# EricssonResearch/Robust-Tracking-MPC-over-Lossy-Networks

Measured on AMD Instinct MI355X. Metric: QP solves/sec (= MPC steps/sec) at batch, higher is better.
Workload: dtype f64

## Files before the change

### robust-tracking-mpc-over-lossy-networks_amd/csrc/tmpc_kernels.hip

```cpp
#ifdef TMPC_HOST_SIM
#include "hip_sim.hpp"
#else
#include <hip/hip_runtime.h>
#endif

#include <algorithm>
#include <cmath>
#include <cstdint>
#include <string>
#include <type_traits>
#include <utility>

#include "tmpc_device.hpp"
#include "tmpc_launch.hpp"
#include "tmpc_wave.hpp"
#include "tmpc_mc_step.hpp"

namespace tmpc {

namespace {

using wv::WAVE;
using wv::fast_rcp;
using wv::readlane_d;
// ... 212 lines not shown
        int ks = 0;
        for (; ks + 1 < nks; ks += 2) {
            fetch(D1, t1, g1);
            multiply(std::integral_constant<int, 0>{}, D0, t0, g0);
            fetch(D0, t0, g0);
            multiply(std::integral_constant<int, NACC - 1>{}, D1, t1, g1);
        }
        if (ks < nks) multiply(std::integral_constant<int, 0>{}, D0, t0, g0);
    }
    static_assert(WaveLds<SH>::RED >= 2 * (SH::NDP + 4), "look-ahead of the MFMA pass stays inside the transposition tile");
    double *mtk = mt + kq * SH::LDM + c;
#pragma unroll
    for (int I = 0; I < NB; ++I)
#pragma unroll
        for (int J = 0; J <= I; ++J)
#pragma unroll
            for (int reg = 0; reg < 4; ++reg) {
                const int row = 16 * I + kq + 4 * reg, col = 16 * J + c;
                double v = acc[0][I * (I + 1) / 2 + J][reg];
                if constexpr (NACC == 2) v += acc[1][I * (I + 1) / 2 + J][reg];
                if (row < NV && col < NV) {
                    mtk[(16 * I + 4 * reg) * SH::LDM + 16 * J] = v;
                    if (I != J) mt[col * SH::LDM + row] = v;
                }
                if (I == IT && row == NV && col < NV) gdr[col] = v;
            }
    wave_lds_fence();
}

template <class SH>
__device__ __forceinline__ void sweep_a_factored(const double *Hct, const double (&s)[SH::RS], const double (&lam)[SH::RS],
                                                 const double *rpw, double (&rs)[SH::RS], double &gap_l, double &rpn_l, double obj_l,
                                                 double *red, double *csums, int lane) {
    constexpr int KC = SH::KC, KT = SH::KT, NCCP = SH::NCCP;
    double acc[KT + KC + 2];
    static_for<SH::FC>([&](auto kc_) {
        constexpr int kc = decltype(kc_)::value;
        const int r = lane + kc * WAVE;
        double hc[KC];
#pragma unroll
        for (int a = 0; a < KC; ++a) hc[a] = Hct[a * NCCP + r];
        double D = 0.0, t = 0.0;
#pragma unroll
        for (int sd = 0; sd < SH::csides(kc); ++sd) {
            constexpr int base = SH::cbase(kc);
            const int i = base + sd;
            const double rsi = fast_rcp(s[i]);
            rs[i] = rsi;
            const double d = lam[i] * rsi;
            const double rpi = rpw[i * WAVE + lane];
            gap_l = fma(s[i], lam[i], gap_l);
            rpn_l = vmax_abs(rpn_l, rpi);
            D += d;
            t = sd ? fma(-d, rpi, t) : fma(d, rpi, t);
        }
#pragma unroll
        for (int a = 0; a < KC; ++a) {
            const double dg = D * hc[a];
#pragma unroll
            for (int b2 = a; b2 < KC; ++b2) acc[col_off<KC>(a) + b2 - a] = kc == 0 ? dg * hc[b2] : fma(dg, hc[b2], acc[col_off<KC>(a) + b2 - a]);
            acc[KT + a] = kc == 0 ? hc[a] * t : fma(hc[a], t, acc[KT + a]);
        }
    });
    acc[KT + KC] = gap_l;
    acc[KT + KC + 1] = obj_l;
    wave_sums_to_lds<SH, KT + KC + 2>(acc, red, csums, lane);
}

struct McNone {};
struct McStepArg {
    const McFused *rec;
    int t;
    uint8_t *gamma_out;
};
template <int FUSED> using McArg = std::conditional_t<FUSED == 1, const McFused *, std::conditional_t<FUSED == 2, McStepArg, McNone>>;
#if defined(TMPC_HOST_SIM)
typedef const McFused *McRecord;
__device__ __forceinline__ McRecord mc_record(const McFused *p) { return p; }
#else
typedef const __attribute__((address_space(4))) McFused *McRecord;
__device__ __forceinline__ McRecord mc_record(const McFused *p) {
    unsigned lo = static_cast<unsigned>(reinterpret_cast<uintptr_t>(p)), hi = static_cast<unsigned>(reinterpret_cast<uintptr_t>(p) >> 32);
    asm volatile("" : "+v"(lo), "+v"(hi));
    lo = __builtin_amdgcn_readfirstlane(lo);
    hi = __builtin_amdgcn_readfirstlane(hi);
    return (McRecord)((static_cast<uintptr_t>(hi) << 32) | lo);
}
#endif

template <int NV, int DP, int DS, int KC, int CP, int CS, int WPB, int FUSED>
__device__ __forceinline__ void solve_body(
    const DeviceQP &qp, const int variant_id, const int64_t B,
    const double *__restrict__ x_k, const double *__restrict__ ref, const uint8_t *__restrict__ variant,
    double *__restrict__ u_nom, double *__restrict__ x_nom0, double *__restrict__ xu_ss,
    double *__restrict__ x_nom, int32_t *__restrict__ status, int32_t *__restrict__ iters,
    const int32_t *ws_in, int32_t *ws_out, unsigned long long *__restrict__ next_item,
    const McArg<FUSED> mc) {
    using SH = Shape<NV, DP, DS, KC, CP, CS, tile_rows(NV, WPB)>;
    using WL = WaveLds<SH>;
    constexpr int RS = SH::RS, FD = SH::FD, FC = SH::FC, NDP = SH::NDP, NCCP = SH::NCCP, KT = SH::KT, WCAP = SH::WCAP, LDG = SH::LDG;
#ifdef TMPC_HOST_SIM
    double *smem = sim::lds<double>();
#else
    extern __shared__ __attribute__((aligned(16))) double smem[];
#endif
    double *wbase = smem;
    double *Hct = wbase + WPB * WL::TOTAL;
    double *Psi = Hct + KC * NCCP;
    double *Hs = Psi + KC * NV;
    double *Hinv = Hs + NV * SH::LDH;
    double *Gt = Hinv + NV * SH::LDH;
    const int grows = 4 * qp.nks;

    const int tid = threadIdx.x;
    const int lane_k = tid & (WAVE - 1);
    int lane = lane_k;
    const int wave = __builtin_amdgcn_readfirstlane(tid >> 6);
    const int nx = qp.nx, nu = qp.nu, N = qp.N, nc = qp.nc;

    for (int i = tid; i < (grows + ZERO_ROWS) * LDG; i += blockDim.x) Gt[i] = (i < grows * LDG) ? qp.Gt[i] : 0.0;
    for (int i = tid; i < KC * NCCP; i += blockDim.x) Hct[i] = qp.Hct[i];
    for (int i = tid; i < KC * NV; i += blockDim.x) Psi[i] = qp.Psi[i];
    for (int i = tid; i < NV * NV; i += blockDim.x) { const int r_ = i / NV, c_ = i - r_ * NV; Hs[r_ * SH::LDH + c_] = qp.Hs[i]; Hinv[r_ * SH::LDH + c_] = qp.Hinv[i]; }
    __syncthreads();

    double *red = wbase + wave * WL::TOTAL;
    double *sums = red + WL::BIG;
    double *csums = sums + WL::SUMS;
    double *Pm = csums + WL::CSUMS;
    double *hw = Pm + WL::PMAT;
    double *vec = hw + WL::HROW;
    double *dtw = red;
    double *Mf = red + WL::RED;
    unsigned *park = reinterpret_cast<unsigned *>(red + WL::POL);
    double *qv = vec;
    double *zv = vec + NV;
    double *cgv = vec + 2 * NV;
    double *xin = vec + 3 * NV;
    double *tv = vec + 3 * NV + 32;
    double *uv = vec + 4 * NV + 32;
    double *dzav = vec + 5 * NV + 32;
    double *dzv = vec + 6 * NV + 32;
    double *czv = vec + 7 * NV + 32;
    double *cdzav = czv + 8;
    double *cdzv = czv + 16;

    const int vmask_k = static_cast<int>(qp.vmask[lane]);
    unsigned vmask = static_cast<unsigned>(vmask_k);
    auto valid = [&](int i) { return ((vmask >> i) & 1u) != 0u; };
#define TMPC_REFRESH() do { lane = fresh(lane_k); vmask = static_cast<unsigned>(fresh(vmask_k)); } while (0)

    const int64_t n_waves = static_cast<int64_t>(gridDim.x) * WPB;
    bool first_item = true;
    for (;;) {
        int64_t b;
        if (first_item) {
            b = B < n_waves ? static_cast<int64_t>(wave) * gridDim.x + blockIdx.x : static_cast<int64_t>(blockIdx.x) * WPB + wave;
            first_item = false;
        } else {
            unsigned long long drawn = ~0ull >> 2;
            if (lane_k == 0) {
                const unsigned long long seen = __hip_atomic_load(next_item, __ATOMIC_RELAXED, __HIP_MEMORY_SCOPE_AGENT);
                if (n_waves + static_cast<int64_t>(seen) < B) drawn = atomicAdd(next_item, 1ull);
            }
            b = n_waves + static_cast<int64_t>((static_cast<unsigned long long>(static_cast<unsigned>(__builtin_amdgcn_readfirstlane(static_cast<int>(drawn >> 32)))) << 32) |
                                               static_cast<unsigned>(__builtin_amdgcn_readfirstlane(static_cast<int>(drawn & 0xffffffffull))));
        }
        if (b >= B) break;
        if (variant != nullptr && variant[b] != variant_id) continue;
        if (variant == nullptr && variant_id != 0) continue;

        int n_steps = 1;
        if constexpr (FUSED == 1) n_steps = mc_record(mc)->T;
        for (int t_mc = 0; t_mc < n_steps; ++t_mc) {
        TMPC_REFRESH();
        if constexpr (FUSED != 0) {
            McRecord mr;
            if constexpr (FUSED == 1) mr = mc_record(mc); else mr = mc_record(mc.rec);
            const double *xh = mr->st.x_hat, *rk = mr->st.ref_k;
            if (lane < nx) { xin[lane] = xh[b * nx + lane]; xin[nx + lane] = rk[b * nx + lane]; }
        } else {
            if (lane < nx) { xin[lane] = x_k[b * nx + lane]; xin[nx + lane] = ref[b * nx + lane]; }
        }
        wave_lds_fence();
        int st = TMPC_STATUS_MAX_ITER;
        int it_done = 0;
#ifdef TMPC_ITERS_TOTAL
        int n_reruns = 0, n_rounds = 0, amb_level = 0;
#endif
        const long long t_begin = qp.ticks ? static_cast<long long>(__builtin_amdgcn_s_memrealtime()) : 0;
#ifdef TMPC_STAMPS
        long long tph[16] = {0, 0, 0, 0, 0, 0, 0, 0, 0, 0, 0, 0, 0, 0, 0, 0};
        long long tlast = __builtin_amdgcn_s_memtime();
#endif
        bool infeasible_par = qp.always_infeasible != 0;
        for (int r = lane; r < qp.npar; r += WAVE) {
            double v = qp.gp0[r];
            for (int c = 0; c < nx; ++c) v += qp.Ep[r * nx + c] * xin[c];
            if (v < -1e-9 * (1.0 + fabs(qp.gp0[r]))) infeasible_par = true;
        }
        infeasible_par = __any(infeasible_par);

        if (lane < NV) {
            double v = 0.0;
            if (lane < qp.nv)
                for (int c = 0; c < nx; ++c) v += qp.F1s[lane * nx + c] * xin[c] + qp.F2s[lane * nx + c] * xin[nx + c];
            qv[lane] = v;
        }
        auto compute_h = [&]() {
            TMPC_REFRESH();
            double hv[RS];
            const double *__restrict__ E0 = qp.Esp + lane;
            constexpr size_t PL = static_cast<size_t>(RS) * WAVE;
            for (int c0 = 0; c0 < nx; c0 += 4) {
                double ev[4][RS];
#pragma unroll
                for (int u = 0; u < 4; ++u) {
                    const size_t cu = static_cast<size_t>(c0 + u < nx ? c0 + u : nx - 1);
#pragma unroll
                    for (int i = 0; i < RS; ++i) ev[u][i] = E0[cu * PL + i * WAVE];
                }
                if (c0 == 0) {
#pragma unroll
                    for (int i = 0; i < RS; ++i) hv[i] = qp.g0p[i * WAVE + lane];
                }
#pragma unroll
                for (int u = 0; u < 4; ++u) {
                    const double xc = c0 + u < nx ? xin[c0 + u] : 0.0;
#pragma unroll
                    for (int i = 0; i < RS; ++i) hv[i] = fma(ev[u][i], xc, hv[i]);
                }
            }
            double hmax = 1.0;
#pragma unroll
            for (int i = 0; i < RS; ++i) {
                if (valid(i)) hmax = fmax(hmax, fabs(hv[i]));
                hw[i * WAVE + lane] = hv[i];
            }
            wave_lds_fence();
            return hmax;
        };
        const double hn = wave_max(compute_h());
        double qn = 1.0;
#pragma unroll
        for (int j = 0; j < NV; ++j) qn = fmax(qn, fabs(qv[j]));
        qn = readlane_d(qn, 0);

        auto unconstrained_minimiser = [&]() {
            TMPC_REFRESH();
            if (lane < NV) {
                double v = 0.0;
#pragma unroll
                for (int j = 0; j < NV; ++j) v -= Hinv[lane * SH::LDH + j] * qv[j];
                zv[lane] = v;
            }
            wave_lds_fence();
            coords_lds<SH>(Psi, zv, czv, lane);
            wave_lds_fence();
        };
        auto raw_slacks = [&](double (&sl)[RS]) {
            TMPC_REFRESH();
            double smin = INFINITY;
            static_for<FD>([&](auto kd_) {
                constexpr int kd = decltype(kd_)::value;
                const double gz = dense_dot<SH, kd>(Gt, grows, zv, lane);
#pragma unroll
                for (int sd = 0; sd < SH::dsides(kd); ++sd) {
                    const int i = SH::dbase(kd) + sd;
                    sl[i] = hw[i * WAVE + lane] - (sd ? -gz : gz);
                    if (valid(i)) smin = vmin(smin, sl[i]);
                }
            });
            static_for<FC>([&](auto kc_) {
                constexpr int kc = decltype(kc_)::value;
                const double gz = fact_dot<SH, kc>(Hct, czv, lane);
#pragma unroll
                for (int sd = 0; sd < SH::csides(kc); ++sd) {
                    const int i = SH::cbase(kc) + sd;
                    sl[i] = hw[i * WAVE + lane] - (sd ? -gz : gz);
                    if (valid(i)) smin = vmin(smin, sl[i]);
                }
            });
            return smin;
        };

        double try_tol = qp.tol;
        const double ncd = static_cast<double>(nc);
        double rdn_last = 0.0;
        bool floor_tried = false;
        bool inW[RS];
        double yall[RS];
        int warm_m = 0;
        {
            unconstrained_minimiser();
            double sl[RS];
            const double smin = wave_min(raw_slacks(sl));
            if (infeasible_par) st = TMPC_STATUS_INFEASIBLE;
            else if (smin >= 0.0) st = TMPC_STATUS_OPTIMAL;
            if (ws_in != nullptr) warm_m = ws_in[b * WS_STRIDE];
        }
        STAMP(0);
        bool try_warm = warm_m > 0 && warm_m <= WCAP;
        int resume_it = -1;
        float *const save = qp.save ? qp.save + (static_cast<size_t>(blockIdx.x) * WPB + wave) * (2 * RS * WAVE) : nullptr;
        bool saved = false;
        bool h_valid = true;
        int ws_m = 0;
        if (st == TMPC_STATUS_MAX_ITER)
        for (;;) {
            bool want_polish = false;
            if (try_warm) {
#pragma unroll
                for (int i = 0; i < RS; ++i) { inW[i] = false; yall[i] = 0.0; }
                for (int k = 0; k < warm_m; ++k) {
                    const int gid = ws_in[b * WS_STRIDE + 1 + k];
#pragma unroll
                    for (int i = 0; i < RS; ++i) inW[i] = inW[i] || (gid == i * WAVE + lane && valid(i));
                }
                want_polish = true;
            } else {
                double s[RS], lam[RS], rs[RS];
                double *rpw = hw;
                int it0 = 0;
                double mu_hand = 0.0;
                if (resume_it >= 0) {
                    if (!h_valid) { compute_h(); h_valid = true; }
                    coords_lds<SH>(Psi, zv, czv, lane);
                    wave_lds_fence();
                    (void)raw_slacks(s);
                    h_valid = false;
                    const double park_mu = WL::PARK_LDS ? *reinterpret_cast<const double *>(park + RS * WAVE) : 0.0;
                    const double park_thr = 1e3 * try_tol * hn;
#pragma unroll
                    for (int i = 0; i < RS; ++i) {
                        const bool vl = valid(i);
                        const double raw = s[i];
                        double sv, lv;
                        if constexpr (WL::PARK_LDS) {
                            lv = fmax(static_cast<double>(__uint_as_float(park[i * WAVE + lane])), 1e-30);
                            sv = raw > park_thr ? raw : fmin(fmax(raw, park_mu * fast_rcp(lv)), park_thr);
                        } else {
                            sv = static_cast<double>(save[i * WAVE + lane]);
                            lv = static_cast<double>(save[(RS + i) * WAVE + lane]);
                            if (raw > 0.0 && fabs(sv - raw) <= 2.5e-7 * sv) sv = raw;
                        }
                        s[i] = vl ? sv : 1.0;
                        lam[i] = vl ? lv : 0.0;
                        rpw[i * WAVE + lane] = vl ? sv - raw : 0.0;
                        rs[i] = 1.0;
                    }
                    wave_lds_fence();
                    it0 = resume_it;
                    resume_it = -1;
                } else {
                    if (!h_valid) { compute_h(); h_valid = true; }
                    unconstrained_minimiser();
                    const double smin = wave_min(raw_slacks(s));
                    const double fl = 0.1 * fmax(-smin, 1.0);
                    h_valid = false;
                    double l1 = 0.0;
#pragma unroll
                    for (int i = 0; i < RS; ++i) l1 = vmax(l1, valid(i) ? -s[i] * qp.cip[i * WAVE + lane] : 0.0);
                    l1 = wave_max(l1);
#ifdef TMPC_LAM0_ONE
                    const double lam0 = l1 < 0.0 ? 2.0 : 1.0;
#else
                    const double lam0 = fmin(fmax(sqrt(sqrt(l1)), 1.0), 1e3);
#endif
#pragma unroll
                    for (int i = 0; i < RS; ++i) {
                        const bool vl = valid(i);
                        const double raw = s[i];
                        s[i] = vl ? fmax(raw, fl) : 1.0;
                        lam[i] = vl ? lam0 : 0.0;
                        rpw[i * WAVE + lane] = vl ? s[i] - raw : 0.0;
                        rs[i] = 1.0;
                    }
                    wave_lds_fence();
                }
                for (int it = it0; it < qp.max_iter; ++it) {
                    it_done = it;
                    STAMP(9);
                    TMPC_REFRESH();
                    double obj_l = 0.0;
                    if (lane < NV) {
                        double v = 0.0;
#pragma unroll
                        for (int j = 0; j < NV; ++j) v += Hs[lane * SH::LDH + j] * zv[j];
                        const double qi = qv[lane], cgi = v + qi;
                        cgv[lane] = cgi;
                        obj_l = zv[lane] * (0.5 * (cgi - qi) + qi);
                    }
                    double gap_l = 0.0, rpn_l = 0.0;
                    if constexpr (FD > 0) sweep_a_dense<SH>(Gt, qp.nks, s, lam, rpw, rs, gap_l, rpn_l, dtw, Mf, sums, lane);
                    if constexpr (KC > 0) {
                        TMPC_REFRESH();
                        sweep_a_factored<SH>(Hct, s, lam, rpw, rs, gap_l, rpn_l, obj_l, red, csums, lane);
                        for (int idx = lane; idx < KC * NV; idx += WAVE) {
                            const int a = idx / NV, j = idx - a * NV;
                            double v = 0.0;
#pragma unroll
                            for (int b2 = 0; b2 < KC; ++b2) {
                                const int lo = a < b2 ? a : b2, hi2 = a < b2 ? b2 : a;
                                v += csums[lo * KC - lo * (lo - 1) / 2 + hi2 - lo] * Psi[b2 * NV + j];
                            }
                            Pm[idx] = v;
                        }
                        double v1 = 0.0;
                        if (lane < NV) {
                            v1 = (FD > 0) ? sums[lane] : 0.0;
#pragma unroll
                            for (int a = 0; a < KC; ++a) v1 += Psi[a * NV + lane] * csums[KT + a];
                        }
                        wave_lds_fence();
                        if (lane < NV) sums[lane] = v1;
                        wave_lds_fence();
                    }
                    double lmax_l = 0.0;
#pragma unroll
                    for (int i = 0; i < RS; ++i) lmax_l = vmax(lmax_l, lam[i]);
                    const bool rp_small = !__any(rpn_l > try_tol * hn);
                    const bool lam_big = __any(lmax_l > 1e10);
                    double gap, obj;
                    if constexpr (KC > 0) {
                        gap = readlane_d(csums[KT + KC], 0);
                        obj = readlane_d(csums[KT + KC + 1], 0);
                    } else {
                        gap = gap_l;
                        obj = obj_l;
                        wv::wave_sum2(gap, obj, lane);
                    }
                    const double mu = gap / ncd;
                    STAMP(1);
                    TMPC_REFRESH();
                    if (!(mu == mu)) { st = TMPC_STATUS_NUMERICAL; break; }
                    const double objs = fmax(fabs(obj), 1.0);
                    STAMP(2);
                    const bool near = rp_small && (gap <= try_tol * objs);
                    if (near || lam_big) {
                        if constexpr (FD > 0) {
                            double accl[NV];
#pragma unroll
                            for (int i = 0; i < NV; ++i) accl[i] = 0.0;
                            static_for<FD>([&](auto kd_) {
                                constexpr int kd = decltype(kd_)::value;
                                const int r = min(lane + kd * WAVE, grows);
                                double dl2 = lam[SH::dbase(kd)];
                                if constexpr (SH::dsides(kd) == 2) dl2 -= lam[SH::dbase(kd) + 1];
#pragma unroll
                                for (int j = 0; j < NV; ++j) accl[j] = fma(Gt[r * LDG + j], dl2, accl[j]);
                                if constexpr (WPB == 8 || TMPC_FENCE_ALL) row_fence();
                            });
                            wave_sums_to_lds<SH, NV>(accl, red, sums + NV, lane);
                        }
                        if constexpr (KC > 0) {
                            double accl[KC];
#pragma unroll
                            for (int a = 0; a < KC; ++a) accl[a] = 0.0;
                            static_for<FC>([&](auto kc_) {
                                constexpr int kc = decltype(kc_)::value;
                                const int r = lane + kc * WAVE;
                                double dl2 = lam[SH::cbase(kc)];
                                if constexpr (SH::csides(kc) == 2) dl2 -= lam[SH::cbase(kc) + 1];
#pragma unroll
                                for (int a = 0; a < KC; ++a) accl[a] = fma(Hct[a * NCCP + r], dl2, accl[a]);
                            });
                            wave_sums_to_lds<SH, KC>(accl, red, csums + KT + KC, lane);
                            double gl = 0.0;
                            if (lane < NV) {
                                gl = (FD > 0) ? sums[NV + lane] : 0.0;
#pragma unroll
                                for (int a = 0; a < KC; ++a) gl += Psi[a * NV + lane] * csums[KT + KC + a];
                            }
                            wave_lds_fence();
                            if (lane < NV) sums[NV + lane] = gl;
                            wave_lds_fence();
                        }
                        double rdn = 0.0, gn = 0.0;
#pragma unroll
                        for (int j = 0; j < NV; ++j) {
                            const double glj = sums[NV + j];
                            rdn = fmax(rdn, fabs(cgv[j] + glj));
                            gn = fmax(gn, fabs(glj));
                        }
                        if (!(rdn == rdn)) { st = TMPC_STATUS_NUMERICAL; break; }
#ifdef TMPC_DEBUG_PRINT
                        if (lane == 0 && b < 2) printf("b %lld it %d rdn %.3e qn %.3e\n", (long long)b, it, rdn, qn);
#endif
                        if (near && rdn <= 1e3 * try_tol * qn) { want_polish = true; rdn_last = readlane_d(rdn, 0); mu_hand = readlane_d(mu, 0); break; }
                        if (lam_big) {
                            const double lmax = wave_max(lmax_l);
                            double hl = 0.0;
#pragma unroll
                            for (int i = 0; i < RS; ++i) {
                                const int sl = i * WAVE + lane;
                                double hv = qp.g0p[sl];
                                for (int c = 0; c < nx; ++c) hv += qp.Esp[static_cast<size_t>(c) * (RS * WAVE) + sl] * xin[c];
                                hl += hv * lam[i];
                            }
                            hl = wave_sum(hl);
                            if (hl < 0.0 && gn <= 1e-6 * lmax) { st = TMPC_STATUS_INFEASIBLE; break; }
                        }
                    }
#ifdef TMPC_DEBUG_PRINT
                    if (lane == 0 && b < 2) printf("b %lld it %d gap %.3e objs %.3e hn %.3e near %d tol %.1e\n", (long long)b, it, gap, objs, hn, (int)near, try_tol);
#endif
                    if (gap <= 1e-15 * objs) {
                        st = TMPC_STATUS_MAX_ITER;
                        if (!floor_tried) { floor_tried = true; want_polish = true; rdn_last = INFINITY; mu_hand = readlane_d(mu, 0); }
                        break;
                    }
                    TMPC_REFRESH();
                    double rhs_i = 0.0;
                    const int li = lane < NV ? lane : 0;
                    {
// ... 109 lines not shown
                                double c1 = 0.0, c2 = 0.0;
#pragma unroll
                                for (int sd = 0; sd < SH::csides(kc); ++sd) side_stats(SH::cbase(kc) + sd, sd == 1, gdz, c1, c2);
#pragma unroll
                                for (int a = 0; a < KC; ++a) {
                                    accc[a] = kc == 0 ? hc[a] * c1 : fma(hc[a], c1, accc[a]);
                                    accc[KC + a] = kc == 0 ? hc[a] * c2 : fma(hc[a], c2, accc[KC + a]);
                                }
                            });
                            accc[2 * KC] = sb1;
                            accc[2 * KC + 1] = sb2;
                            wave_sums_to_lds<SH, 2 * KC + 2>(accc, red, csums + KT, lane);
                            sb1 = readlane_d(csums[KT + 2 * KC], 0);
                            sb2 = readlane_d(csums[KT + 2 * KC + 1], 0);
                        } else {
                            wv::wave_sum2(sb1, sb2, lane);
                        }
                        rho_aff = wave_max(rho_aff);
                        if (lane < NV) {
                            if constexpr (FD > 0) { v2 = sums[lane]; v3 = sums[NV + lane]; }
                            if constexpr (KC > 0) {
#pragma unroll
                                for (int a = 0; a < KC; ++a) { v2 += Psi[a * NV + lane] * csums[KT + a]; v3 += Psi[a * NV + lane] * csums[KT + KC + a]; }
                            }
                        }
                    }
                    STAMP(4);
                    TMPC_REFRESH();
                    const double aaff = rho_aff > 1.0 ? 1.0 / rho_aff : 1.0;
                    const double mu_aff = (gap + aaff * sb1 + aaff * aaff * sb2) / ncd;
                    double sigma = mu_aff / mu;
                    sigma = fmin(sigma * sigma * sigma, 1.0);
                    const double smu = sigma * mu;
                    if constexpr (NV > wv::DPP_ROW && wv::DPP_ROW > 0) {
                        if (lane < NV) tv[lane] = rhs_i + v2 - smu * v3;
                        wave_lds_fence();
                        wv::rows32_resolve<NV, SH::LDM>(Mf, tv, dzv, lane);
                    } else {
                        double mrow[NV];
#pragma unroll
                        for (int j = 0; j < NV; ++j) mrow[j] = Mf[li * SH::LDM + j];
                        const double mdinv = Mf[li * SH::LDM + NV];
                        double bb = (lane < NV) ? rhs_i + v2 - smu * v3 : 0.0;
                        lanes_forward<NV>(mrow, bb, lane);
                        const double xl = lanes_backsub_lane<NV>(mrow, bb, mdinv, lane);
                        if (lane < NV) dzv[lane] = xl;
                    }
                    wave_lds_fence();
                    if constexpr (KC > 0) { coords_lds<SH>(Psi, dzv, cdzv, lane); wave_lds_fence(); }
                    STAMP(5);
                    TMPC_REFRESH();
                    double om = (1.0 - aaff) * (1.0 - aaff);
                    om = fmin(fmax(om, 1e-4), 1e-2);
                    const double tau = 1.0 - om;
                    double rho = 0.0;
                    {
                        auto side_step = [&](int i, bool neg, double gdz) {
                            const double rpi = rpw[i * WAVE + lane];
                            const double dsk = neg ? gdz - rpi : -rpi - gdz;
                            const double t1 = fma(lam[i], dsk, wv_[i] - smu);
                            const double dlk = valid(i) ? fma(-t1, rs[i], -lam[i]) : 0.0;
                            const double rl = valid(i) ? rcp1(lam[i]) : 0.0;
                            rho = vmax(rho, vmax(-dsk * rs[i], -dlk * rl));
                            rs[i] = dsk;
                            wv_[i] = dlk;
                        };
                        static_for<FD>([&](auto kd_) {
                            constexpr int kd = decltype(kd_)::value;
                            const double gdz = dense_dot<SH, kd>(Gt, grows, dzv, lane);
#pragma unroll
                            for (int sd = 0; sd < SH::dsides(kd); ++sd) side_step(SH::dbase(kd) + sd, sd == 1, gdz);
                            if constexpr (WPB == 8 || TMPC_FENCE_ALL) row_fence();
                        });
                        static_for<FC>([&](auto kc_) {
                            constexpr int kc = decltype(kc_)::value;
                            const double gdz = fact_dot<SH, kc>(Hct, cdzv, lane);
#pragma unroll
                            for (int sd = 0; sd < SH::csides(kc); ++sd) side_step(SH::cbase(kc) + sd, sd == 1, gdz);
                        });
                    }
                    rho = wave_max(rho);
                    const double alpha = rho > tau ? tau / rho : 1.0;
                    const double oma = 1.0 - alpha;
#pragma unroll
                    for (int i = 0; i < RS; ++i) {
                        s[i] = fma(alpha, rs[i], s[i]);
                        lam[i] = fma(alpha, wv_[i], lam[i]);
                        rpw[i * WAVE + lane] *= oma;
                    }
                    if (lane < NV) zv[lane] += alpha * dzv[lane];
                    wave_lds_fence();
                    it_done = it + 1;
                    STAMP(6);
                }
                TMPC_REFRESH();
#ifdef TMPC_DEBUG_PRINT
                if (lane == 0 && b < 2) printf("b %lld ipm exit: it_done %d st %d want_polish %d tol %.1e it0 %d\n", (long long)b, it_done, st, (int)want_polish, try_tol, it0);
#endif
#pragma unroll
                for (int i = 0; i < RS; ++i) { inW[i] = valid(i) && (lam[i] > s[i]); yall[i] = lam[i]; }
#ifdef TMPC_ITERS_TOTAL
                if (want_polish && amb_level == 0) {
                    amb_level = 9;
#pragma unroll
                    for (int i = 0; i < RS; ++i) {
                        if (valid(i)) {
                            const double lr = fabs(log10(lam[i] / s[i]));
                            const int k = lr < 1.0 ? 1 : (lr < 2.0 ? 2 : (lr < 3.0 ? 3 : (lr < 4.0 ? 4 : (lr < 6.0 ? 6 : 9))));
                            amb_level = k < amb_level ? k : amb_level;
                        }
                    }
                    amb_level = -static_cast<int>(wave_max(-static_cast<double>(amb_level)));
                }
#endif
                if constexpr (WL::PARK_LDS) {
                    if (want_polish) {
#pragma unroll
                        for (int i = 0; i < RS; ++i) park[i * WAVE + lane] = __float_as_uint(static_cast<float>(lam[i]));
                        if (lane == 0) *reinterpret_cast<double *>(park + RS * WAVE) = mu_hand;
                        saved = true;
                        wave_lds_fence();
                    }
                } else if (save != nullptr && want_polish) {
                    bool amb = false;
#pragma unroll
                    for (int i = 0; i < RS; ++i) amb = amb || (valid(i) && lam[i] < 100.0 * s[i] && s[i] < 100.0 * lam[i]);
                    saved = __ballot(amb) != 0ull;
                    if (saved) {
#pragma unroll
                        for (int i = 0; i < RS; ++i) {
                            save[i * WAVE + lane] = static_cast<float>(s[i]);
                            save[(RS + i) * WAVE + lane] = static_cast<float>(lam[i]);
                        }
                    }
                }
            }
            if (!want_polish) break;
            bool ok = false;
            if (!h_valid) { compute_h(); h_valid = true; }
            {
                double *GW = red;
                double *T = GW + WCAP * SH::LDW;
                double *yv = T + NV * SH::LDT;
                double *dyv = yv + WCAP;
                int *Widx = reinterpret_cast<int *>(dyv + WCAP);
                double *zpv = dzav;
                if (lane < NV) zpv[lane] = zv[lane];
                wave_lds_fence();
                const int max_rounds = (try_tol == qp.tol && saved && !try_warm) ? 4 : 10;
                int loose_retries = 0;
                for (int round = 0; round < max_rounds + loose_retries && !ok; ++round) {
#ifdef TMPC_ITERS_TOTAL
                    ++n_rounds;
#endif
                    TMPC_REFRESH();
                    int m = 0;
                    {
                        int cnt = 0;
#pragma unroll
                        for (int i = 0; i < RS; ++i) cnt += __popcll(__ballot(inW[i]));
                        if (cnt > WCAP) {
                            double ym = 0.0;
#pragma unroll
                            for (int i = 0; i < RS; ++i) ym = fmax(ym, inW[i] ? yall[i] : 0.0);
                            double thr = 1e-14 * wave_max(ym);
                            for (int tries = 0; tries < 14 && cnt > WCAP; ++tries) {
                                thr *= 10.0;
                                cnt = 0;
#pragma unroll
                                for (int i = 0; i < RS; ++i) {
                                    inW[i] = inW[i] && (yall[i] == 0.0 || yall[i] > thr);
                                    cnt += __popcll(__ballot(inW[i]));
                                }
                            }
                        }
                    }
#pragma unroll
                    for (int i = 0; i < RS; ++i) {
                        const unsigned long long bal = __ballot(inW[i]);
                        const int pos = m + __popcll(bal & ((1ull << lane) - 1ull));
                        if (inW[i] && pos < WCAP) { Widx[pos] = i * WAVE + lane; yv[pos] = yall[i]; }
                        m += __popcll(bal);
                    }
                    wave_lds_fence();
                    STAMP(10);
                    if (m > WCAP) break;
                    if (m == 0) {
                        if (lane < NV) {
                            double v = 0.0;
#pragma unroll
                            for (int j = 0; j < NV; ++j) v -= Hinv[lane * SH::LDH + j] * qv[j];
                            zpv[lane] = v;
                        }
                        wave_lds_fence();
                    } else {
                        for (int idx = lane; idx < m * NV; idx += WAVE) {
                            const int k = idx / NV, j = idx - k * NV;
                            const int gid = Widx[k];
                            bool dense;
                            int fs;
                            double sgn;
                            side_info<SH>(gid >> 6, dense, fs, sgn);
                            const int r = fs * WAVE + (gid & 63);
                            double v = 0.0;
                            if (dense) {
                                if constexpr (FD > 0) v = Gt[r * LDG + j];
                            } else {
                                if constexpr (KC > 0) {
#pragma unroll
                                    for (int a = 0; a < KC; ++a) v += Hct[a * NCCP + r] * Psi[a * NV + j];
                                }
                            }
                            GW[k * SH::LDW + j] = sgn * v;
                        }
                        wave_lds_fence();
                        for (int idx = lane; idx < NV * m; idx += WAVE) {
                            const int i = idx / m, k = idx - i * m;
                            double v = 0.0;
#pragma unroll
                            for (int j = 0; j < NV; ++j) v += Hinv[i * SH::LDH + j] * GW[k * SH::LDW + j];
                            T[i * SH::LDT + k] = v;
                        }
                        wave_lds_fence();
                        STAMP(11);
                        auto solve_working_set = [&]<int MC>(std::integral_constant<int, MC>) -> bool {
                        TMPC_REFRESH();
                        double srow[MC], sdinv = 1.0;
                        {
                            double gw[NV];
                            const int la = lane < m ? lane : 0;
#pragma unroll
                            for (int j = 0; j < NV; ++j) gw[j] = GW[la * SH::LDW + j];
                            double sdiag = 0.0;
#pragma unroll
                            for (int c2 = 0; c2 < MC; ++c2) {
                                double v = 0.0;
#pragma unroll
                                for (int j = 0; j < NV; ++j) v += gw[j] * T[j * SH::LDT + c2];
                                const bool in = lane < m && c2 < m;
                                srow[c2] = in ? v : ((c2 == lane) ? 1.0 : 0.0);
                                if (c2 == lane && in) sdiag = v;
                            }
                            const double dmax = wave_max(sdiag);
#pragma unroll
                            for (int c2 = 0; c2 < MC; ++c2) if (c2 == lane && lane < m) srow[c2] += 1e-11 * dmax;
                        }
                        {
                            double bdummy = 0.0;
                            if (!lanes_factor<MC>(srow, bdummy, sdinv, lane)) return false;
                        }
                        STAMP(12);
                        double dz_prev = 0.0;
                        for (int stp = 0; stp < 12; ++stp) {
                            TMPC_REFRESH();
                            if (lane < NV) {
                                double v = qv[lane];
#pragma unroll
                                for (int j = 0; j < NV; ++j) v += Hs[lane * SH::LDH + j] * zpv[j];
                                for (int k = 0; k < m; ++k) v += GW[k * SH::LDW + lane] * yv[k];
                                tv[lane] = v;
                            }
                            wave_lds_fence();
                            if (lane < NV) {
                                double v = 0.0;
#pragma unroll
                                for (int j = 0; j < NV; ++j) v += Hinv[lane * SH::LDH + j] * tv[j];
                                uv[lane] = v;
                            }
                            wave_lds_fence();
                            double bb = 0.0;
                            if (lane < m) {
                                double gz = 0.0, gt = 0.0;
#pragma unroll
                                for (int j = 0; j < NV; ++j) { const double g = GW[lane * SH::LDW + j]; gz += g * zpv[j]; gt += g * uv[j]; }
                                bb = gz - hw[Widx[lane]] - gt;
                            }
                            lanes_forward<MC>(srow, bb, lane);
                            const double dyl = lanes_backsub_lane<MC>(srow, bb, sdinv, lane);
                            if (lane < m) { dyv[lane] = dyl; yv[lane] += dyl; }
                            wave_lds_fence();
                            double dzl = 0.0, zl = 0.0;
                            if (lane < NV) {
                                double v = uv[lane];
                                for (int k = 0; k < m; ++k) v += T[lane * SH::LDT + k] * dyv[k];
                                zl = zpv[lane] - v;
                                zpv[lane] = zl;
                                dzl = fabs(v);
                            }
                            wave_lds_fence();
                            const double dzn = wave_max(dzl), zn = fmax(wave_max(fabs(zl)), 1.0);
                            if (stp >= 1) {
                                const double rho = dzn / fmax(dz_prev, 1e-300);
                                if (dzn <= 1e-14 * zn || (loose_retries == 0 && rho < 0.5 && dzn * rho <= 0.5e-15 * zn)) break;
                            }
                            dz_prev = dzn;
                        }
                            return true;
                        };
                        bool fact_ok;
                        if (m <= 12) fact_ok = solve_working_set(std::integral_constant<int, 12>{});
                        else if (WCAP == 24 || m <= 24) fact_ok = solve_working_set(std::integral_constant<int, 24>{});
                        else fact_ok = solve_working_set(std::integral_constant<int, WCAP>{});
                        if (!fact_ok) break;
                    }
                    STAMP(13);
                    TMPC_REFRESH();
                    double ymax = 1.0;
                    for (int k = 0; k < m; ++k) ymax = fmax(ymax, fabs(yv[k]));
                    int nviol = 0, nneg = 0, nloose = 0;
                    double yloose = INFINITY;
                    {
                        if constexpr (KC > 0) { coords_lds<SH>(Psi, zpv, cdzav, lane); wave_lds_fence(); }
                        int mm = 0;
                        auto check_side = [&](int i, double gz) {
                            const double hk = hw[i * WAVE + lane];
                            const double rr = gz - hk;
                            const unsigned long long bal = __ballot(inW[i]);
                            const int pos = mm + __popcll(bal & ((1ull << lane) - 1ull));
                            mm += __popcll(bal);
                            const double hi = fmax(fabs(hk), 1.0);
                            const bool viol = valid(i) && !inW[i] && rr > 1e-12 * hi;
                            const bool loose = inW[i] && fabs(rr) > 1e-11 * hi;
                            bool neg = false;
                            if (inW[i]) { yall[i] = yv[pos < WCAP ? pos : 0]; neg = yall[i] < -1e-10 * ymax; }
                            nviol += __popcll(__ballot(viol));
                            nneg += __popcll(__ballot(neg));
                            nloose += __popcll(__ballot(loose));
                            if (loose && !neg) yloose = fmin(yloose, yall[i]);
                            if (neg) { inW[i] = false; yall[i] = 0.0; }
                            if (viol) { inW[i] = true; yall[i] = 0.0; }
                        };
                        static_for<FD>([&](auto kd_) {
                            constexpr int kd = decltype(kd_)::value;
                            const double gz = dense_dot<SH, kd>(Gt, grows, zpv, lane);
#pragma unroll
                            for (int sd = 0; sd < SH::dsides(kd); ++sd) check_side(SH::dbase(kd) + sd, sd ? -gz : gz);
                        });
                        static_for<FC>([&](auto kc_) {
                            constexpr int kc = decltype(kc_)::value;
                            const double gz = fact_dot<SH, kc>(Hct, cdzav, lane);
#pragma unroll
                            for (int sd = 0; sd < SH::csides(kc); ++sd) check_side(SH::cbase(kc) + sd, sd ? -gz : gz);
                        });
                    }
                    wave_lds_fence();
                    STAMP(14);
#ifdef TMPC_DEBUG_PRINT
                    if (lane == 0 && b < 2) {
                        printf("b %lld warm %d tol %.1e it %d round %d m %d nviol %d nneg %d nloose %d ymax %.3e W:", (long long)b, (int)try_warm, try_tol, it_done, round, m, nviol, nneg, nloose, ymax);
                        for (int k = 0; k < m && k < WCAP; ++k) printf(" %d(%.2e)", Widx[k], yv[k]);
                        printf("\n");
                    }
#endif
                    if (try_warm && !(nviol == 0 && nneg == 0) && (round >= 2 || nviol + nneg > 6 || nloose != 0)) break;
                    if (nloose != 0 && nviol == 0 && nneg == 0) {
                        if (try_warm) break;
                        if (loose_retries < 2) { ++loose_retries; continue; }
                        const double ymin = wave_min(yloose);
#pragma unroll
                        for (int i = 0; i < RS; ++i)
                            if (inW[i] && yall[i] == ymin) { inW[i] = false; yall[i] = 0.0; }
                        continue;
                    }
                    if (nviol == 0 && nneg == 0) {
                        ok = true;
                        if (lane < NV) zv[lane] = zpv[lane];
                        ws_m = m;
                        if (ws_out != nullptr && lane < m) ws_out[b * WS_STRIDE + 1 + lane] = Widx[lane];
                        wave_lds_fence();
                    }
                }
            }
            STAMP(7);
            if (ok) { st = TMPC_STATUS_OPTIMAL; break; }
            if (try_warm) { try_warm = false; continue; }
            if (try_tol <= 1e-12) { st = (rdn_last <= 1e-9 * qn) ? TMPC_STATUS_OPTIMAL : TMPC_STATUS_MAX_ITER; break; }
            try_tol *= 1e-2;
            if (saved) resume_it = it_done;
            saved = false;
#ifdef TMPC_ITERS_TOTAL
            ++n_reruns;
#endif
        }
#ifdef TMPC_DEBUG_PRINT
        if (lane == 0 && (st == TMPC_STATUS_MAX_ITER || st == TMPC_STATUS_NUMERICAL) && nx == 4)
            printf("NONOPT b %lld st %d it %d tol %.1e x %a %a %a %a r %a\n", (long long)b, st, it_done, try_tol, xin[0], xin[1], xin[2], xin[3], xin[4]);
#endif
        if (ws_out != nullptr && lane == 0) ws_out[b * WS_STRIDE] = ws_m;

        TMPC_REFRESH();
        const bool good = st < TMPC_STATUS_INFEASIBLE;
        const double nanv = __longlong_as_double(0x7ff8000000000000ll);
        wave_lds_fence();
        const double *zo = zv;
        if (qp.Tzs != nullptr) {
            double *zf = hw;
            for (int i = lane; i < qp.nvf; i += WAVE) {
                double v = 0.0;
                for (int c = 0; c < nx; ++c) v += qp.Txf[i * nx + c] * xin[c];
                for (int j = 0; j < qp.nv; ++j) v += qp.Tzs[i * qp.nv + j] * zv[j];
                zf[i] = v;
            }
            zo = zf;
        } else if (lane < NV) {
            zv[lane] = (lane < qp.nv) ? qp.Dv[lane] * zv[lane] : 0.0;
        }
        wave_lds_fence();
        for (int i = lane; i < N * nu; i += WAVE) u_nom[b * N * nu + i] = good ? zo[i] : nanv;
        if (lane < nx + nu) {
            double v = 0.0;
            for (int j = 0; j < qp.nth; ++j) v += qp.Mth[lane * qp.nth + j] * zo[qp.off_theta + j];
            if (xu_ss) xu_ss[b * (nx + nu) + lane] = good ? v : nanv;
        }
        if (lane < nx) {
            const double x0 = (qp.off_x0 >= 0) ? zo[qp.off_x0 + lane] : xin[lane];
            if (x_nom0) x_nom0[b * nx + lane] = good ? x0 : nanv;
            tv[lane] = x0;
        }
        if (x_nom) {
            wave_lds_fence();
            if (lane < nx) x_nom[b * (N + 1) * nx + lane] = good ? tv[lane] : nanv;
            for (int i = 0; i < N; ++i) {
                double v = 0.0;
                if (lane < nx) {
                    for (int j = 0; j < nx; ++j) v += qp.A[lane * nx + j] * tv[j];
                    for (int j = 0; j < nu; ++j) v += qp.B[lane * nu + j] * zo[i * nu + j];
                }
                wave_lds_fence();
                if (lane < nx) { tv[lane] = v; x_nom[b * (N + 1) * nx + (i + 1) * nx + lane] = good ? v : nanv; }
                wave_lds_fence();
            }
        }
#ifdef TMPC_ITERS_TOTAL
        if (lane == 0) { status[b] = st; iters[b] = it_done + 100 * n_reruns + 10000 * n_rounds + 1000000 * amb_level; }
#else
        if (lane == 0) { status[b] = st; iters[b] = it_done; }
#endif
        if (qp.ticks && lane == 0) qp.ticks[b] = static_cast<long long>(__builtin_amdgcn_s_memrealtime()) - t_begin;
#ifdef TMPC_STAMPS
        STAMP(8);
        if (b == 0 && lane == 0 && qp.dbg) { for (int p_ = 0; p_ < 16; ++p_) qp.dbg[p_] = tph[p_]; }
#endif
        wave_lds_fence();
        if constexpr (FUSED != 0) {
            TMPC_REFRESH();
            __builtin_amdgcn_fence(__ATOMIC_SEQ_CST, "workgroup");
            McRecord mr;
            int t_now = t_mc, t_all = n_steps;
            uint8_t *gamma_out = nullptr;
            if constexpr (FUSED == 1) mr = mc_record(mc);
            else { mr = mc_record(mc.rec); t_now = mc.t; t_all = mr->T; gamma_out = mc.gamma_out; }
            const int t_next = t_now + 1 < t_all ? t_now + 1 : t_now;
            const double *rseq = mr->ref_seq;
            const bool alive = mcstep::mc_step_wave(mr->m, mr->st, t_now, t_all, b, rseq[t_now], rseq[t_next], u_nom, x_nom0, xu_ss, status,
                                                    iters, *reinterpret_cast<double (*)[mcstep::V_COUNT][mcstep::MAXN]>(red), lane, gamma_out);
            __builtin_amdgcn_fence(__ATOMIC_SEQ_CST, "workgroup");
            wave_lds_fence();
            if (!alive) break;
        }
        }
    }
}

template <int NV, int DP, int DS, int KC, int CP, int CS, int WPB>
__global__ __launch_bounds__(WAVE *WPB, 1) void solve_kernel(
    const DeviceQP qp, const int variant_id, const int64_t B,
    const double *__restrict__ x_k, const double *__restrict__ ref, const uint8_t *__restrict__ variant,
    double *__restrict__ u_nom, double *__restrict__ x_nom0, double *__restrict__ xu_ss,
    double *__restrict__ x_nom, int32_t *__restrict__ status, int32_t *__restrict__ iters,
    const int32_t *ws_in, int32_t *ws_out, unsigned long long *__restrict__ next_item) {
    solve_body<NV, DP, DS, KC, CP, CS, WPB, 0>(qp, variant_id, B, x_k, ref, variant, u_nom, x_nom0, xu_ss, x_nom, status, iters, ws_in, ws_out,
                                                   next_item, McNone{});
}
template <int NV, int DP, int DS, int KC, int CP, int CS, int WPB>
__global__ __launch_bounds__(WAVE *WPB, 1) void closed_loop_kernel(
    const DeviceQP qp, const int64_t B, double *__restrict__ u_nom, double *__restrict__ x_nom0, double *__restrict__ xu_ss,
    int32_t *__restrict__ status, int32_t *__restrict__ iters, int32_t *ws, unsigned long long *__restrict__ next_item,
    const McFused *mc) {
    solve_body<NV, DP, DS, KC, CP, CS, WPB, 1>(qp, 0, B, nullptr, nullptr, nullptr, u_nom, x_nom0, xu_ss, nullptr, status, iters, ws, ws,
                                               next_item, mc);
}
template <int NV, int DP, int DS, int KC, int CP, int CS, int WPB>
__global__ __launch_bounds__(WAVE *WPB, 1) void closed_loop_step_kernel(
    const DeviceQP qp, const int variant_id, const int64_t B, const uint8_t *__restrict__ variant,
    double *__restrict__ u_nom, double *__restrict__ x_nom0, double *__restrict__ xu_ss,
    int32_t *__restrict__ status, int32_t *__restrict__ iters, int32_t *ws, unsigned long long *__restrict__ next_item,
    const McStepArg mc) {
    solve_body<NV, DP, DS, KC, CP, CS, WPB, 2>(qp, variant_id, B, nullptr, nullptr, variant, u_nom, x_nom0, xu_ss, nullptr, status, iters, ws, ws,
                                               next_item, mc);
}

template <class SH>
constexpr size_t kernel_lds_bytes(int wpb, int grows) {
    return sizeof(double) * (static_cast<size_t>(SH::LDG) * (grows + ZERO_ROWS) + SH::KC * SH::NCCP + SH::KC * SH::NV + 2 * SH::NV * SH::LDH +
                             static_cast<size_t>(wpb) * WaveLds<SH>::TOTAL);
}
template <int DP, int DS>
constexpr int design_rows() { return (DP + DS) * WAVE <= 64 ? (DP + DS) * WAVE : ((DP + DS) * WAVE * 3) / 4; }
template <int NV, int DP, int DS, int KC, int CP, int CS>
constexpr int waves_per_block() {
    constexpr int gr = design_rows<DP, DS>();
    if (NV <= 12 && !(NV > 8 && DS >= 4) && kernel_lds_bytes<Shape<NV, DP, DS, KC, CP, CS, tile_rows(NV, 8)>>(8, gr) <= 160 * 1024) return 8;
    using SH = Shape<NV, DP, DS, KC, CP, CS, tile_rows(NV, 4)>;
    return kernel_lds_bytes<SH>(4, gr) <= 160 * 1024 ? 4 : (kernel_lds_bytes<SH>(3, gr) <= 160 * 1024 ? 3 : 2);
}

#if defined(TMPC_ONE_SHAPE)
#define TMPC_APPLY(X, ...) X(__VA_ARGS__)
#define TMPC_SHAPES(X) TMPC_APPLY(X, TMPC_ONE_SHAPE)
#elif defined(TMPC_ONLY_BENCH)
#define TMPC_SHAPES(X) X(11, 1, 0, 5, 4, 0)
#elif defined(TMPC_SIM_SHAPES_N20)
#define TMPC_SHAPES(X) X(22, 2, 0, 5, 4, 0) X(26, 2, 0, 4, 7, 0)
#elif defined(TMPC_SIM_SHAPES_EXT)
#define TMPC_SHAPES(X) X(11, 1, 0, 5, 4, 0) X(15, 1, 0, 4, 7, 0)
#elif defined(TMPC_SIM_SHAPES)
#define TMPC_SHAPES(X) X(11, 1, 0, 5, 4, 0) X(8, 0, 2, 0, 0, 0)
#else
#define TMPC_SHAPES(X) \
    X(8, 0, 2, 0, 0, 0) X(8, 0, 4, 0, 0, 0) X(12, 0, 2, 0, 0, 0) X(12, 0, 4, 0, 0, 0) X(16, 0, 2, 0, 0, 0) X(16, 0, 4, 0, 0, 0) \
    X(11, 1, 0, 5, 4, 0) X(12, 1, 0, 5, 4, 0) X(22, 2, 0, 5, 4, 0) X(24, 2, 0, 5, 4, 0) X(15, 1, 0, 4, 7, 0) X(16, 1, 0, 4, 7, 0) X(26, 2, 0, 4, 7, 0)
#endif

template <int NV, int... R>
struct ShapeTag {
    static constexpr int WPB = waves_per_block<NV, R...>();
    using SH = Shape<NV, R..., tile_rows(NV, WPB)>;
};

template <class Ret, class F>
Ret with_shape(const KernelShape &s, Ret miss, F &&f) {
#define TMPC_CASE(A, B_, C, D, E, F_) \
    if (s.nvp == A && s.dp == B_ && s.ds == C && s.kcp == D && s.cp == E && s.cs == F_) return f(ShapeTag<A, B_, C, D, E, F_>{});
    TMPC_SHAPES(TMPC_CASE)
#undef TMPC_CASE
    return miss;
}

template <class T, int FUSED>
constexpr bool instantiated() {
#if !defined(TMPC_HOST_SIM)
    return true;
#elif defined(TMPC_SIM_SHAPES_EXT)
    return FUSED == 2;
#elif defined(TMPC_SIM_SHAPES)
    return FUSED == 0 || (FUSED == 1 && std::is_same_v<T, ShapeTag<11, 1, 0, 5, 4, 0>>);
#else
    return FUSED != 2;
#endif
}

template <int FUSED, int... S>
hipError_t launch_wpb(ShapeTag<S...>, const DeviceQP &qp, int variant_id, const BatchIO &io, const int32_t *ws_in, int32_t *ws_out,
                      WorkCounter *wc, int n_cu, hipStream_t stream, McArg<FUSED> mc) {
    using SH = typename ShapeTag<S...>::SH;
    constexpr int WPB = ShapeTag<S...>::WPB;
    static_assert(SH::RS <= 32, "validity mask is one 32-bit word per lane");
    const size_t lds = kernel_lds_bytes<SH>(WPB, 4 * qp.nks);
    if (lds > 160 * 1024) return hipErrorInvalidValue;
    const unsigned blocks = static_cast<unsigned>(std::max<int64_t>(1, std::min<int64_t>(io.B, n_cu)));
    unsigned long long *next_item = nullptr;
    if (const hipError_t e = next_word(wc, stream, &next_item); e != hipSuccess) return e;
    if constexpr (FUSED == 1)
        return launch_grid(closed_loop_kernel<S..., WPB>, blocks, WAVE * WPB, lds, stream, qp, io.B, io.u_nom, io.x_nom0, io.xu_ss, io.status,
// ... 83 lines not shown
```

Baseline: 11.74 million.

## Prefetch per-item loads early, skip redundant unconstrained test, and draw next item ahead

Issues the E/g0 plane loads, F1/F2/Ep coefficients and state inputs before the LDS fence so the global-memory latency overlaps with setup. When no warm start or infeasibility is present, the initial unconstrained feasibility test is skipped and folded into the first cold-start round. Warm-start ids are read once per lane and broadcast with readlane, and the next work item's atomic is issued during the output phase. This adds register pressure from the held prefetch buffers and restructures the control flow in a few places.

```diff
diff --git a/robust-tracking-mpc-over-lossy-networks_amd/csrc/tmpc_kernels.hip b/robust-tracking-mpc-over-lossy-networks_amd/csrc/tmpc_kernels.hip
--- a/robust-tracking-mpc-over-lossy-networks_amd/csrc/tmpc_kernels.hip
+++ b/robust-tracking-mpc-over-lossy-networks_amd/csrc/tmpc_kernels.hip
@@ -388,17 +388,24 @@
 
     const int64_t n_waves = static_cast<int64_t>(gridDim.x) * WPB;
     bool first_item = true;
+    auto draw = [&]() {
+        unsigned long long drawn = ~0ull >> 2;
+        if (lane_k == 0) {
+            const unsigned long long seen = __hip_atomic_load(next_item, __ATOMIC_RELAXED, __HIP_MEMORY_SCOPE_AGENT);
+            if (n_waves + static_cast<int64_t>(seen) < B) drawn = atomicAdd(next_item, 1ull);
+        }
+        return drawn;
+    };
+    bool drawn_ahead = false;
+    unsigned long long drawn_next = 0;
     for (;;) {
         int64_t b;
         if (first_item) {
             b = B < n_waves ? static_cast<int64_t>(wave) * gridDim.x + blockIdx.x : static_cast<int64_t>(blockIdx.x) * WPB + wave;
             first_item = false;
         } else {
-            unsigned long long drawn = ~0ull >> 2;
-            if (lane_k == 0) {
-                const unsigned long long seen = __hip_atomic_load(next_item, __ATOMIC_RELAXED, __HIP_MEMORY_SCOPE_AGENT);
-                if (n_waves + static_cast<int64_t>(seen) < B) drawn = atomicAdd(next_item, 1ull);
-            }
+            const unsigned long long drawn = drawn_ahead ? drawn_next : draw();
+            drawn_ahead = false;
             b = n_waves + static_cast<int64_t>((static_cast<unsigned long long>(static_cast<unsigned>(__builtin_amdgcn_readfirstlane(static_cast<int>(drawn >> 32)))) << 32) |
                                                static_cast<unsigned>(__builtin_amdgcn_readfirstlane(static_cast<int>(drawn & 0xffffffffull))));
         }
@@ -410,45 +417,37 @@
         if constexpr (FUSED == 1) n_steps = mc_record(mc)->T;
         for (int t_mc = 0; t_mc < n_steps; ++t_mc) {
         TMPC_REFRESH();
-        if constexpr (FUSED != 0) {
-            McRecord mr;
-            if constexpr (FUSED == 1) mr = mc_record(mc); else mr = mc_record(mc.rec);
-            const double *xh = mr->st.x_hat, *rk = mr->st.ref_k;
-            if (lane < nx) { xin[lane] = xh[b * nx + lane]; xin[nx + lane] = rk[b * nx + lane]; }
-        } else {
-            if (lane < nx) { xin[lane] = x_k[b * nx + lane]; xin[nx + lane] = ref[b * nx + lane]; }
-        }
-        wave_lds_fence();
-        int st = TMPC_STATUS_MAX_ITER;
-        int it_done = 0;
-#ifdef TMPC_ITERS_TOTAL
-        int n_reruns = 0, n_rounds = 0, amb_level = 0;
-#endif
-        const long long t_begin = qp.ticks ? static_cast<long long>(__builtin_amdgcn_s_memrealtime()) : 0;
-#ifdef TMPC_STAMPS
-        long long tph[16] = {0, 0, 0, 0, 0, 0, 0, 0, 0, 0, 0, 0, 0, 0, 0, 0};
-        long long tlast = __builtin_amdgcn_s_memtime();
-#endif
-        bool infeasible_par = qp.always_infeasible != 0;
-        for (int r = lane; r < qp.npar; r += WAVE) {
-            double v = qp.gp0[r];
-            for (int c = 0; c < nx; ++c) v += qp.Ep[r * nx + c] * xin[c];
-            if (v < -1e-9 * (1.0 + fabs(qp.gp0[r]))) infeasible_par = true;
-        }
-        infeasible_par = __any(infeasible_par);
-
-        if (lane < NV) {
-            double v = 0.0;
-            if (lane < qp.nv)
-                for (int c = 0; c < nx; ++c) v += qp.F1s[lane * nx + c] * xin[c] + qp.F2s[lane * nx + c] * xin[nx + c];
-            qv[lane] = v;
-        }
-        auto compute_h = [&]() {
+        struct HLoad { double g0[RS], ev[4][RS]; };
+        auto h_issue = [&](HLoad &hl) {
+            TMPC_REFRESH();
+            const double *__restrict__ E0 = qp.Esp + lane;
+            constexpr size_t PL = static_cast<size_t>(RS) * WAVE;
+#pragma unroll
+            for (int u = 0; u < 4; ++u) {
+                const size_t cu = static_cast<size_t>(u < nx ? u : nx - 1);
+#pragma unroll
+                for (int i = 0; i < RS; ++i) hl.ev[u][i] = E0[cu * PL + i * WAVE];
+            }
+#pragma unroll
+            for (int i = 0; i < RS; ++i) hl.g0[i] = qp.g0p[i * WAVE + lane];
+        };
+        auto h_finish = [&](const HLoad &hl) {
             TMPC_REFRESH();
             double hv[RS];
             const double *__restrict__ E0 = qp.Esp + lane;
             constexpr size_t PL = static_cast<size_t>(RS) * WAVE;
-            for (int c0 = 0; c0 < nx; c0 += 4) {
+#pragma unroll
+            for (int i = 0; i < RS; ++i) hv[i] = hl.g0[i];
+            auto add_planes = [&](const double (&ev)[4][RS], int c0) {
+#pragma unroll
+                for (int u = 0; u < 4; ++u) {
+                    const double xc = c0 + u < nx ? xin[c0 + u] : 0.0;
+#pragma unroll
+                    for (int i = 0; i < RS; ++i) hv[i] = fma(ev[u][i], xc, hv[i]);
+                }
+            };
+            add_planes(hl.ev, 0);
+            for (int c0 = 4; c0 < nx; c0 += 4) {
                 double ev[4][RS];
 #pragma unroll
                 for (int u = 0; u < 4; ++u) {
@@ -456,16 +455,7 @@
 #pragma unroll
                     for (int i = 0; i < RS; ++i) ev[u][i] = E0[cu * PL + i * WAVE];
                 }
-                if (c0 == 0) {
-#pragma unroll
-                    for (int i = 0; i < RS; ++i) hv[i] = qp.g0p[i * WAVE + lane];
-                }
-#pragma unroll
-                for (int u = 0; u < 4; ++u) {
-                    const double xc = c0 + u < nx ? xin[c0 + u] : 0.0;
-#pragma unroll
-                    for (int i = 0; i < RS; ++i) hv[i] = fma(ev[u][i], xc, hv[i]);
-                }
+                add_planes(ev, c0);
             }
             double hmax = 1.0;
 #pragma unroll
@@ -476,7 +466,74 @@
             wave_lds_fence();
             return hmax;
         };
-        const double hn = wave_max(compute_h());
+        auto compute_h = [&]() {
+            HLoad hl;
+            h_issue(hl);
+            return h_finish(hl);
+        };
+        double xk_l = 0.0, ref_l = 0.0;
+        if constexpr (FUSED != 0) {
+            McRecord mr;
+            if constexpr (FUSED == 1) mr = mc_record(mc); else mr = mc_record(mc.rec);
+            const double *xh = mr->st.x_hat, *rk = mr->st.ref_k;
+            if (lane < nx) { xk_l = xh[b * nx + lane]; ref_l = rk[b * nx + lane]; }
+        } else {
+            if (lane < nx) { xk_l = x_k[b * nx + lane]; ref_l = ref[b * nx + lane]; }
+        }
+        int warm_m = 0;
+        if (ws_in != nullptr) warm_m = ws_in[b * WS_STRIDE];
+        HLoad hl0;
+        h_issue(hl0);
+        double f1_l[4] = {0.0, 0.0, 0.0, 0.0}, f2_l[4] = {0.0, 0.0, 0.0, 0.0}, ep_l[4] = {0.0, 0.0, 0.0, 0.0}, gp0_l = 0.0;
+        if (lane < NV && lane < qp.nv) {
+#pragma unroll
+            for (int c = 0; c < 4; ++c) {
+                const int cc = c < nx ? c : nx - 1;
+                f1_l[c] = qp.F1s[lane * nx + cc];
+                f2_l[c] = qp.F2s[lane * nx + cc];
+            }
+        }
+        if (lane < qp.npar) {
+            gp0_l = qp.gp0[lane];
+#pragma unroll
+            for (int c = 0; c < 4; ++c) ep_l[c] = qp.Ep[lane * nx + (c < nx ? c : nx - 1)];
+        }
+        if (lane < nx) { xin[lane] = xk_l; xin[nx + lane] = ref_l; }
+        wave_lds_fence();
+        int st = TMPC_STATUS_MAX_ITER;
+        int it_done = 0;
+#ifdef TMPC_ITERS_TOTAL
+        int n_reruns = 0, n_rounds = 0, amb_level = 0;
+#endif
+        const long long t_begin = qp.ticks ? static_cast<long long>(__builtin_amdgcn_s_memrealtime()) : 0;
+#ifdef TMPC_STAMPS
+        long long tph[16] = {0, 0, 0, 0, 0, 0, 0, 0, 0, 0, 0, 0, 0, 0, 0, 0};
+        long long tlast = __builtin_amdgcn_s_memtime();
+#endif
+        bool infeasible_par = qp.always_infeasible != 0;
+        for (int r = lane; r < qp.npar; r += WAVE) {
+            const bool first = r < WAVE;
+            const double g = first ? gp0_l : qp.gp0[r];
+            double v = g;
+#pragma unroll
+            for (int c = 0; c < 4; ++c)
+                if (c < nx) v += (first ? ep_l[c] : qp.Ep[r * nx + c]) * xin[c];
+            for (int c = 4; c < nx; ++c) v += qp.Ep[r * nx + c] * xin[c];
+            if (v < -1e-9 * (1.0 + fabs(g))) infeasible_par = true;
+        }
+        infeasible_par = __any(infeasible_par);
+
+        if (lane < NV) {
+            double v = 0.0;
+            if (lane < qp.nv) {
+#pragma unroll
+                for (int c = 0; c < 4; ++c)
+                    if (c < nx) v += f1_l[c] * xin[c] + f2_l[c] * xin[nx + c];
+                for (int c = 4; c < nx; ++c) v += qp.F1s[lane * nx + c] * xin[c] + qp.F2s[lane * nx + c] * xin[nx + c];
+            }
+            qv[lane] = v;
+        }
+        const double hn = wave_max(h_finish(hl0));
         double qn = 1.0;
 #pragma unroll
         for (int j = 0; j < NV; ++j) qn = fmax(qn, fabs(qv[j]));
@@ -526,14 +583,13 @@
         bool floor_tried = false;
         bool inW[RS];
         double yall[RS];
-        int warm_m = 0;
-        {
+        const bool tested_here = infeasible_par || warm_m > 0;
+        if (tested_here) {
             unconstrained_minimiser();
             double sl[RS];
             const double smin = wave_min(raw_slacks(sl));
             if (infeasible_par) st = TMPC_STATUS_INFEASIBLE;
             else if (smin >= 0.0) st = TMPC_STATUS_OPTIMAL;
-            if (ws_in != nullptr) warm_m = ws_in[b * WS_STRIDE];
         }
         STAMP(0);
         bool try_warm = warm_m > 0 && warm_m <= WCAP;
@@ -548,8 +604,9 @@
             if (try_warm) {
 #pragma unroll
                 for (int i = 0; i < RS; ++i) { inW[i] = false; yall[i] = 0.0; }
+                const int gid_l = lane < warm_m ? ws_in[b * WS_STRIDE + 1 + lane] : -1;
                 for (int k = 0; k < warm_m; ++k) {
-                    const int gid = ws_in[b * WS_STRIDE + 1 + k];
+                    const int gid = __builtin_amdgcn_readlane(gid_l, k);
 #pragma unroll
                     for (int i = 0; i < RS; ++i) inW[i] = inW[i] || (gid == i * WAVE + lane && valid(i));
                 }
@@ -589,14 +646,18 @@
                     it0 = resume_it;
                     resume_it = -1;
                 } else {
+                    double ci[RS];
+#pragma unroll
+                    for (int i = 0; i < RS; ++i) ci[i] = qp.cip[i * WAVE + lane];
                     if (!h_valid) { compute_h(); h_valid = true; }
                     unconstrained_minimiser();
                     const double smin = wave_min(raw_slacks(s));
+                    if (!tested_here && smin >= 0.0) { st = TMPC_STATUS_OPTIMAL; break; }
                     const double fl = 0.1 * fmax(-smin, 1.0);
                     h_valid = false;
                     double l1 = 0.0;
 #pragma unroll
-                    for (int i = 0; i < RS; ++i) l1 = vmax(l1, valid(i) ? -s[i] * qp.cip[i * WAVE + lane] : 0.0);
+                    for (int i = 0; i < RS; ++i) l1 = vmax(l1, valid(i) ? -s[i] * ci[i] : 0.0);
                     l1 = wave_max(l1);
 #ifdef TMPC_LAM0_ONE
                     const double lam0 = l1 < 0.0 ? 2.0 : 1.0;
@@ -1012,6 +1073,9 @@
                 for (int round = 0; round < max_rounds + loose_retries && !ok; ++round) {
 #ifdef TMPC_ITERS_TOTAL
                     ++n_rounds;
+#endif
+#ifdef TMPC_STAMPS
+                    tph[15] += 1;
 #endif
                     TMPC_REFRESH();
                     int m = 0;
@@ -1252,6 +1316,10 @@
         const bool good = st < TMPC_STATUS_INFEASIBLE;
         const double nanv = __longlong_as_double(0x7ff8000000000000ll);
         wave_lds_fence();
+        double dv_l = 0.0, mth_l = 0.0;
+        if (qp.Tzs == nullptr && lane < NV && lane < qp.nv) dv_l = qp.Dv[lane];
+        if (lane < nx + nu && qp.nth > 0) mth_l = qp.Mth[lane * qp.nth];
+        if constexpr (FUSED != 1) { drawn_next = draw(); drawn_ahead = true; }
         const double *zo = zv;
         if (qp.Tzs != nullptr) {
             double *zf = hw;
@@ -1263,13 +1331,14 @@
             }
             zo = zf;
         } else if (lane < NV) {
-            zv[lane] = (lane < qp.nv) ? qp.Dv[lane] * zv[lane] : 0.0;
+            zv[lane] = (lane < qp.nv) ? dv_l * zv[lane] : 0.0;
         }
         wave_lds_fence();
         for (int i = lane; i < N * nu; i += WAVE) u_nom[b * N * nu + i] = good ? zo[i] : nanv;
         if (lane < nx + nu) {
             double v = 0.0;
-            for (int j = 0; j < qp.nth; ++j) v += qp.Mth[lane * qp.nth + j] * zo[qp.off_theta + j];
+            if (qp.nth > 0) v += mth_l * zo[qp.off_theta];
+            for (int j = 1; j < qp.nth; ++j) v += qp.Mth[lane * qp.nth + j] * zo[qp.off_theta + j];
             if (xu_ss) xu_ss[b * (nx + nu) + lane] = good ? v : nanv;
         }
         if (lane < nx) {
```

Measured after the change: 11.78 million, median of 6. No clear change (+0.4%).
